# turnDeep/Computational-Chemistry-AI

Measured on AMD Instinct MI355X. Metric: scf_iterations_per_sec, higher is better.
Workload: dtype f64

## Files before the change

### computational-chemistry-ai_amd/csrc/mi355scf.hip

```cpp

#include <hip/hip_runtime.h>
#include <algorithm>
#include <chrono>
#include <cmath>
#include <cstdarg>
#include <cstdint>
#include <cstdio>
#include <cstring>
#include <numeric>
#include <string>
#include <thread>
#include <type_traits>
#include <mutex>
#include <map>
#include <unordered_map>
#include <vector>

#include "../../include/mi355scf.h"
#include "rys_tables.h"

#define LMAX 4
#define LMAX_1E 3
#define NPC ((LMAX + 1) * (LMAX + 2) / 2)
#define BLK 8
// ... 343 lines not shown
    int opt_jk_pipe = -1;
    int opt_ao_order = 1;
    int opt_ket_cluster = 1;
    int opt_xf_mlds = 0;
    int opt_rys_qpw_maxcomp = 256;
    double opt_rys_qpw_maxprim = 4.0;
    int opt_xf_qpw_max = 40;
    int opt_work_mb = 2048;
    int opt_grad_work_mb = 1024;
    int opt_vmat_fold_mt = 3;
    int opt_rys_fine = 1;
    int opt_eri_fused = 0;
    int opt_task_table = 1;
    int opt_prim_lds = 0;
    int opt_xcd_map = 1;
    int opt_df_batch_max = 0;
    int ao_order = 0;
    int *d_perm = nullptr, *d_iperm = nullptr;
    std::vector<int> perm, iperm;
    int opt_vmat_xcd = 1;
    int opt_vmat_wgs = 0;
    int opt_sp2_direct = 0;
    double *d_xt_scratch = nullptr;
};

static inline int pc_index(int la, int lb) { return la * (la + 1) / 2 + lb; }
static inline int ne_of(int la, int lb) { int n = 0; for (int e = la; e <= la + lb; e++) n += ncart(e); return n; }

static double gaussian_int(int n, double a) { return std::tgamma((n + 1) * 0.5) / (2.0 * std::pow(a, (n + 1) * 0.5)); }

static int set_tile_order(mi_ctx *c, int order)
{
    if (c->ao_order == order) return 0;
    const int nbas = c->nbas;
    std::vector<int> seq(nbas);
    std::iota(seq.begin(), seq.end(), 0);
    if (order == 1) std::stable_sort(seq.begin(), seq.end(), [&](int a, int b) { return c->shells[a].l < c->shells[b].l; });
    c->perm.assign(std::max(c->nao, 1), 0);
    c->iperm.assign(std::max(c->nao, 1), 0);
    int pos = 0;
    for (int s_ : seq) {
        ShellH &S = c->shells[s_];
        S.ao = pos;
        for (int m = 0; m < 2 * S.l + 1; m++) { c->perm[S.ao_nat + m] = pos + m; c->iperm[pos + m] = S.ao_nat + m; }
        pos += 2 * S.l + 1;
    }
// ... 241 lines not shown
    void *ptrs[] = {c->d_prim, c->d_M, c->d_tile_table, c->d_tile_off, c->d_tile_I, c->d_runs, c->d_tiles, c->d_segs, c->d_wave_seg,
                    c->d_tile_present};
    for (void *p : ptrs) if (p) dev_free(p);
    c->d_tile_present = nullptr;
    c->d_prim = c->d_M = nullptr; c->d_tile_table = nullptr; c->d_tile_off = nullptr; c->d_tile_I = nullptr;
    c->d_runs = nullptr; c->d_tiles = nullptr; c->d_segs = nullptr; c->d_wave_seg = nullptr;
    c->eri_ready = false;
}

extern "C" int mi_eri_release(mi_ctx *c)
{
    if (!c) return fail("mi_eri_release: null context");
    hipSetDevice(c->device);
    free_eri(c);
    return 0;
}

extern "C" void mi_ctx_destroy(mi_ctx *c)
{
    if (!c) return;
    hipSetDevice(c->device);
    free_eri(c);
    void *ptrs[] = {c->d_env, c->d_bas, c->d_atm, c->d_shell_ao, c->d_c2s, c->d_rys_cheb, c->d_herm_r, c->d_herm_w,
                    c->d_Dpad, c->d_Jacc, c->d_Kacc, c->d_red, c->d_shell_xyz, c->d_xt_scratch, c->d_perm, c->d_iperm,
                    c->d_mDpad, c->d_mJacc, c->d_mKacc};
    for (void *p : ptrs) if (p) dev_free(p);
    {
        HostStash &H = g_stash[c->device & 15];
        std::lock_guard<std::mutex> g(H.mu);
        if (c->h_M.capacity() > H.h_M.capacity()) H.h_M.swap(c->h_M);
        if (c->h_prim.capacity() > H.h_prim.capacity()) H.h_prim.swap(c->h_prim);
        if (c->tiles.capacity() > H.tiles.capacity()) H.tiles.swap(c->tiles);
        if (c->tile_off.capacity() > H.tile_off.capacity()) H.tile_off.swap(c->tile_off);
    }
    delete c;
}

extern "C" int mi_ctx_nao(const mi_ctx *c) { return c ? c->nao : -1; }

extern "C" int mi_set_option(mi_ctx *c, const char *key, double value)
{
    if (!c || !key) return fail("mi_set_option: null argument");
    std::string k(key);
    if (k == "runmax") c->opt_runmax = (int)value;
    else if (k == "omega") {
        if (!(value >= 0.0) || !std::isfinite(value)) return fail("mi_set_option: omega must be finite and >= 0");
        c->opt_omega = value;
    }
    else if (k == "jk_waves") c->opt_jk_waves = (int)value;
    else if (k == "jk_nt") c->opt_jk_nt = (int)value;
    else if (k == "jk_pipe") c->opt_jk_pipe = (int)value;
    else if (k == "jk_dpp") c->opt_jk_dpp = (int)value;
    else if (k == "jk_kjlt") c->opt_jk_kjlt = (int)value;
    else if (k == "grad_live") c->opt_grad_live = (int)value;
    else if (k == "grad_rows") c->opt_grad_rows = (int)value;
    else if (k == "grad_rows_min") c->opt_grad_rows_min = (int)value;
    else if (k == "grad_rows_g32") g_rows_g32 = (int)value;
    else if (k == "jk_cache_mb") c->opt_jk_cache_mb = (int)value;
    else if (k == "jk_pair") c->opt_jk_pair = (int)value;
    else if (k == "jk_multi_batch") c->opt_jk_multi_batch = (int)value;
    else if (k == "sp2_direct") c->opt_sp2_direct = (int)value;
    else if (k == "vmat_wgs") c->opt_vmat_wgs = (int)value;
    else if (k == "vmat_xcd") c->opt_vmat_xcd = (int)value;
    else if (k == "tri_tiles") c->opt_tri_tiles = (int)value;
    else if (k == "ao_order") c->opt_ao_order = (int)value;
    else if (k == "ket_cluster") c->opt_ket_cluster = (int)value;
    else if (k == "xcd_map") c->opt_xcd_map = (int)value;
    else if (k == "prim_lds") c->opt_prim_lds = (int)value;
    else if (k == "task_table") c->opt_task_table = (int)value;
    else if (k == "eri_fused") c->opt_eri_fused = (int)value;
    else if (k == "rys_fine") c->opt_rys_fine = (int)value;
    else if (k == "df_batch_max") {
        if (!(value >= 0.0) || value > 2147483647.0) return fail("mi_set_option: df_batch_max must be in [0, 2^31)");
        c->opt_df_batch_max = (int)value;
    }
    else if (k == "vmat_fold_mt") c->opt_vmat_fold_mt = (int)value;
    else if (k == "work_mb") c->opt_work_mb = (int)value;
    else if (k == "grad_work_mb") c->opt_grad_work_mb = (int)value;
    else if (k == "rys_qpw_maxcomp") c->opt_rys_qpw_maxcomp = (int)value;
    else if (k == "rys_qpw_maxprim") c->opt_rys_qpw_maxprim = value;
    else if (k == "xf_qpw_max") c->opt_xf_qpw_max = (int)value;
    else if (k == "xf_mlds") c->opt_xf_mlds = (int)value;
    else if (k == "eri_tpq") c->opt_eri_tpq = (int)value;
    else if (k == "tpq_maxprim") c->opt_tpq_maxprim = value;
// ... 3433 lines not shown
extern "C" int mi_diis_dots_dev_n(mi_ctx *c, const double *d_hist_e, const double *d_e, int n, int64_t len, double *d_out, void *stream)
{
    if (!c || n < 1 || n > 64 || len < 1 || !d_out) return fail("mi_diis_dots_dev_n: bad argument");
    hipLaunchKernelGGL(diis_dots_kernel, dim3(n, DIIS_NS), dim3(256), 0, (hipStream_t)stream, d_hist_e, d_e, (size_t)len, d_out);
    HIPCHK(hipGetLastError());
    return 0;
}

extern "C" int mi_diis_dots_dev(mi_ctx *c, const double *d_hist_e, const double *d_e, int n, double *d_out, void *stream)
{
    if (!c) return fail("mi_diis_dots_dev: bad argument");
    return mi_diis_dots_dev_n(c, d_hist_e, d_e, n, (int64_t)c->nao * c->nao, d_out, stream);
}

#define DIIS_MAXM 16
__device__ __forceinline__ double lane_bcast(double x, int l)
{
    const int ls = __builtin_amdgcn_readfirstlane(l);
    const long long b = __double_as_longlong(x);
    const unsigned lo = (unsigned)__builtin_amdgcn_readlane((int)(b & 0xffffffffll), ls);
    const unsigned hi = (unsigned)__builtin_amdgcn_readlane((int)(b >> 32), ls);
    return __longlong_as_double((long long)(((unsigned long long)hi << 32) | lo));
}
__global__ __launch_bounds__(64) void diis_solve_kernel(const double *__restrict__ part, int m, int slot, int space, double *B, double *__restrict__ coef)
{
    __shared__ double A[DIIS_MAXM + 1][DIIS_MAXM + 3];
    __shared__ double X[DIIS_MAXM + 1];
    const int t = threadIdx.x;
    const int n = m + 1;
    double bold[DIIS_MAXM];
#pragma unroll
    for (int j = 0; j < DIIS_MAXM; j++) bold[j] = (t >= 1 && t <= m && j < m) ? B[(t - 1) * space + j] : 0.0;
    double dot = 0.0;
    if (t < m) {
        double pq[DIIS_NS];
#pragma unroll
        for (int q = 0; q < DIIS_NS; q++) pq[q] = part[t * DIIS_NS + q];
#pragma unroll
        for (int q = 0; q < DIIS_NS; q++) dot += pq[q];
        B[slot * space + t] = dot;
        B[t * space + slot] = dot;
        X[t] = dot;
    }
    __syncthreads();
    if (t < n) {
#pragma unroll
        for (int j = 0; j <= DIIS_MAXM; j++) {
            double v = 0.0;
            if (j < n) {
                if (t == 0) v = (j == 0) ? 0.0 : 1.0;
                else if (j == 0) v = 1.0;
                else if (t - 1 == slot) v = X[j - 1];
                else if (j - 1 == slot) v = X[t - 1];
                else v = bold[j - 1];
            }
            A[t][j] = v;
        }
        A[t][n] = (t == 0) ? 1.0 : 0.0;
    }
    __syncthreads();
    bool ok = true;
    for (int k = 0; k < n && ok; k++) {
        double val = (t >= k && t < n) ? fabs(A[t][k]) : -1.0;
        int p = t;
        for (int o = 32; o > 0; o >>= 1) {
            const double v2 = __shfl_xor(val, o);
            const int p2 = __shfl_xor(p, o);
            if (v2 > val || (v2 == val && p2 < p)) { val = v2; p = p2; }
        }
        if (!(val > 0.0) || !isfinite(val)) { ok = false; break; }
        if (p != k && t <= n) { const double x = A[k][t]; A[k][t] = A[p][t]; A[p][t] = x; }
        __syncthreads();
        if (t > k && t < n) {
            const double f = A[t][k] / A[k][k];
            for (int j = k; j <= n; j++) A[t][j] = fma(-f, A[k][j], A[t][j]);
        }
        __syncthreads();
    }
    if (ok) {
        for (int i = n - 1; i >= 0; i--) {
            if (t == i) X[i] = A[i][n] / A[i][i];
            __syncthreads();
            const double xi = X[i];
            if (!isfinite(xi)) ok = false;
            if (t < i) A[t][n] = fma(-A[t][i], xi, A[t][n]);
            __syncthreads();
        }
    }
    if (t >= 1 && t <= m) coef[t - 1] = ok ? X[t] : ((t - 1) == slot ? 1.0 : 0.0);
}

extern "C" int mi_diis_solve(mi_ctx *c, const double *d_part, int m, int slot, int space, double *d_B, double *d_coef, void *stream)
{
    if (!c || !d_part || !d_B || !d_coef || m < 1 || m > DIIS_MAXM || space < m || slot < 0 || slot >= m) return fail("mi_diis_solve: bad argument");
    hipLaunchKernelGGL(diis_solve_kernel, dim3(1), dim3(64), 0, (hipStream_t)stream, d_part, m, slot, space, d_B, d_coef);
    HIPCHK(hipGetLastError());
    return 0;
}

__global__ void diis_combine_dev_kernel(const double *hist, const double *coef, int n, size_t nn, double *out)
{
    size_t idx = (size_t)blockIdx.x * blockDim.x + threadIdx.x;
    if (idx >= nn) return;
    const MI_CONST_AS double *cf = as_const(coef);
    double s = 0.0;
    for (int i = 0; i < n; i++) s = fma(cf[i], hist[(size_t)i * nn + idx], s);
    out[idx] = s;
}

extern "C" int mi_diis_combine_dev_n(mi_ctx *c, const double *d_hist, const double *d_coef, int n, int64_t len, double *d_out, void *stream)
{
    if (!c || !d_hist || !d_coef || !d_out || n < 1 || n > DIIS_MAXM || len < 1) return fail("mi_diis_combine_dev_n: bad argument");
// ... 3432 lines not shown
    double s = 0.0;
    if (idx < (size_t)n * n) {
        int r = (int)(idx / n), cidx = (int)(idx - (size_t)r * n);
        double v = M[idx] - M[(size_t)cidx * n + r];
        E[idx] = v;
        s = v * v;
    }
    for (int o = 32; o > 0; o >>= 1) s += __shfl_xor(s, o);
    if ((threadIdx.x & 63) == 0) sh[threadIdx.x >> 6] = s;
    __syncthreads();
    if (threadIdx.x == 0) part[blockIdx.x] = (sh[0] + sh[1]) + (sh[2] + sh[3]);
}

extern "C" int mi_commutator_norm(mi_ctx *c, const double *d_M, double *d_E, double *d_part, void *stream)
{
    if (!c || !d_M || !d_E || !d_part) return fail("mi_commutator_norm: null argument");
    int n = c->nao;
    hipLaunchKernelGGL(commutator_norm_kernel, dim3((unsigned)(((size_t)n * n + 255) / 256)), dim3(256), 0, (hipStream_t)stream, d_M, n, d_E,
                       d_part);
    HIPCHK(hipGetLastError());
    return 0;
}

#define VM_T 64
#define VM_KS 64
#define VM_PAD 2
__global__ __launch_bounds__(256) void xc_vmat_kernel(const double *__restrict__ A, const double *__restrict__ W, int nao, int64_t ng,
                                                      int64_t kchunk, double *C, int xcd_order)
{
    __shared__ double Pa[VM_T][VM_KS + VM_PAD], Pb[VM_T][VM_KS + VM_PAD];
    const int nt = (nao + VM_T - 1) / VM_T, ntt = nt * nt;
    const int L = (int)blockIdx.x;
    int tile, split;
    if (xcd_order) { split = (L & 7) + 8 * (L / (8 * ntt)); tile = (L >> 3) % ntt; }
    else { tile = L % ntt; split = L / ntt; }
    const int m0 = (tile / nt) * VM_T, n0 = (tile % nt) * VM_T;
    const int64_t kbeg = (int64_t)split * kchunk, kend = min(ng, kbeg + kchunk);
    const int wave = threadIdx.x >> 6, lane = threadIdx.x & 63;
    const int qm = (wave >> 1) * 32, qn = (wave & 1) * 32;
    const bool va0 = m0 + qm < nao, va1 = m0 + qm + 16 < nao, vb0 = n0 + qn < nao, vb1 = n0 + qn + 16 < nao;
    d4_t acc[2][2];
#pragma unroll
    for (int a = 0; a < 2; a++)
#pragma unroll
        for (int b = 0; b < 2; b++) acc[a][b] = d4_t{0.0, 0.0, 0.0, 0.0};
    constexpr int PER = VM_T * VM_KS / 256;
// ... 664 lines not shown
```

### computational-chemistry-ai_amd/python/mi355scf/engine.py

```python
import ctypes
import os

import numpy as np
import torch

_HERE = os.path.dirname(os.path.abspath(__file__))
_CSRC = os.path.normpath(os.path.join(_HERE, "..", "..", "csrc"))
LIB_PATH = os.path.join(_CSRC, "libmi355scf.so")
_lib = None


class EngineError(RuntimeError):
    pass


class EngineOutOfMemory(EngineError):

    def __init__(self, msg, need_bytes, free_bytes):
        super().__init__(msg)
        self.need_bytes, self.free_bytes = need_bytes, free_bytes


MI_ERR_NOMEM = -2

# ... 74 lines not shown
        L.mi_sp2_iterate.argtypes = [vp, vp, vp, ctypes.c_int, ctypes.c_double, ctypes.c_int, vp, vp, ctypes.POINTER(vp), vp]
        L.mi_sp2_iterate_pingpong.argtypes = [vp, vp, vp, ctypes.c_int, ctypes.c_double, vp, ctypes.POINTER(vp), ctypes.POINTER(vp), vp]
        L.mi_sp2_iterate_planned.argtypes = [vp, vp, vp, vp, ctypes.c_int, dp, ctypes.c_double, vp, ctypes.POINTER(vp), ctypes.POINTER(vp), vp]
        L.mi_grad_1e.argtypes = [vp, vp, vp, vp, vp]
        L.mi_grad_eri.argtypes = [vp, vp, ctypes.c_double, vp, vp]
        L.mi_grad_eri_spin.argtypes = [vp, vp, vp, ctypes.c_double, vp, vp]
        L.mi_grad_eri_sharded.argtypes = [vp, vp, vp, ctypes.c_double, vp, ctypes.c_int, ctypes.c_int, vp]
        L.mi_grad_eri_pairs.argtypes = [vp, vp, vp, ctypes.c_double, vp, dp, ctypes.c_int, vp, ctypes.c_int, ctypes.c_int, vp]
        L.mi_grad_eri_xpairs.argtypes = [vp, vp, vp, ctypes.c_double, vp, dp, ctypes.c_int, vp, dp, ctypes.POINTER(ctypes.c_int), ctypes.c_int,
                                         vp, ctypes.c_int, ctypes.c_int, vp]
        L.mi_eri_get_memory.argtypes = [vp, ctypes.POINTER(ctypes.c_int64), ctypes.POINTER(ctypes.c_int64)]
        L.mi_eri_release.argtypes = [vp]
        L.mi_tile_store_allocations.restype = ctypes.c_int64
        L.mi_tile_store_allocations.argtypes = [ctypes.c_int64]
        L.mi_eri_read_quartet.argtypes = [vp, ctypes.c_int, ctypes.c_int, ctypes.c_int, ctypes.c_int, dp]
        L.mi_schwarz_get.argtypes = [vp, dp]
        L.mi_df_build.argtypes = [vp, vp, vp, vp, vp]
        L.mi_df_grad.argtypes = [vp, vp, vp, vp, vp, ctypes.c_int, ctypes.c_int, vp]
        L.mi_reduce_blocks.argtypes = [vp]
        L.mi_plan_shards.argtypes = [ctypes.c_int, dp, ctypes.c_double, ctypes.c_int, ctypes.POINTER(ctypes.c_int64),
                                     ctypes.POINTER(ctypes.c_int64)]
        L.mi_fock_energy.argtypes = [vp, vp, vp, vp, vp, vp, ctypes.c_double, vp, vp, vp]
        L.mi_commutator_norm.argtypes = [vp, vp, vp, vp, vp]
        L.mi_c2s_table.argtypes = [ctypes.c_int, dp]
        L.mi_rys_roots_host.argtypes = [ctypes.c_int, ctypes.c_double, dp, dp]
        L.mi_pcm_pairs.argtypes = [vp, ctypes.c_int, ip]
        L.mi_pcm_eval.argtypes = [vp, vp, ctypes.c_int, vp, ctypes.c_int, i64, vp, vp]
        L.mi_pcm_grad.argtypes = [vp, vp, ctypes.c_int, vp, ctypes.c_int, vp, vp, vp, vp]
        L.mi_pcm_potential.argtypes = [vp, vp, ctypes.c_int, i64, vp, vp, vp, vp, vp]
        L.mi_pcm_fock_chunks.argtypes = [ctypes.c_int, i64]
        L.mi_pcm_fock.argtypes = [vp, vp, ctypes.c_int, i64, vp, ctypes.c_double, ctypes.c_int, vp, vp, vp]
        ci = ctypes.c_int
        L.mi_fci_gather_d.argtypes = [vp, ci, ci, ci, ci, ci, ci, vp, ci, vp, ci, vp, vp]
        L.mi_fci_gather_sigma.argtypes = [vp, ci, ci, ci, ci, ci, ci, vp, ci, vp, vp, vp]
        L.mi_fci_hdiag.argtypes = [vp, vp, vp, ci, vp, ci, vp, ci, vp, vp]
        L.mi_cc_amp_update.argtypes = [vp, vp, vp, vp, vp, vp, vp, ci, ci, vp, vp, vp]
        L.mi_cc_t_blocks.argtypes = [ci]
        L.mi_cc_t_energy.argtypes = [vp, ci, ci, ci, vp, vp, vp, vp, vp, vp, vp, vp, vp]
        L.mi_rohf_fock.argtypes = [vp, vp, i64, ci, ci, ci, vp, vp, vp, vp]
        _lib = L
    return _lib


def plan_shards(nao, qblk, tol, nranks):
    q = np.ascontiguousarray(qblk, dtype=np.float64)
    b = np.zeros(nranks, dtype=np.int64)
# ... 533 lines not shown
        _check(lib().mi_sp2_iterate_planned(self._h, F.data_ptr(), A.data_ptr(), B.data_ptr(), nit, _dp(coef), float(out_scale),
                                            tr.data_ptr(), ctypes.byref(out), ctypes.byref(res), self._stream()))
        return (A if res.value == A.data_ptr() else B), (out.value - tr.data_ptr()) // 8

    def build_fock(self, D, h, kscale, F, part, with_k=True, vxc_unsym=None):
        if not self.eri_ready:
            self.prepare_eri()
        assert D.is_contiguous() and F.is_contiguous() and part.numel() == self.reduce_blocks and part.is_contiguous()
        assert vxc_unsym is None or vxc_unsym.is_contiguous()
        with torch.cuda.device(self.device):
            _check(lib().mi_build_fock(self._h, D.data_ptr(), h.data_ptr(), vxc_unsym.data_ptr() if vxc_unsym is not None else None,
                                       int(bool(with_k)), float(kscale), F.data_ptr(), part.data_ptr(), self._stream()))
        return F

    def fock_energy(self, h, J, K, Vxc, D, kscale, F, part):
        assert part.numel() == self.reduce_blocks and part.is_contiguous()
        _check(lib().mi_fock_energy(self._h, h.data_ptr(), J.data_ptr(), K.data_ptr() if K is not None else None,
                                    Vxc.data_ptr() if Vxc is not None else None, D.data_ptr(), float(kscale), F.data_ptr(),
                                    part.data_ptr(), self._stream()))

    def commutator_norm(self, M, E, part):
        assert part.numel() == self.reduce_blocks and part.is_contiguous()
        _check(lib().mi_commutator_norm(self._h, M.data_ptr(), E.data_ptr(), part.data_ptr(), self._stream()))

    def diis_errvec(self, sdf, out):
        _check(lib().mi_diis_errvec(self._h, sdf.data_ptr(), out.data_ptr(), self._stream()))

    def diis_combine(self, hist, coef, out):
        c = np.ascontiguousarray(coef, dtype=np.float64)
        _check(lib().mi_diis_combine(self._h, hist.data_ptr(), _dp(c), len(c), out.data_ptr(), self._stream()))

    def diis_dots_dev(self, hist_e, e, n, out):
        _check(lib().mi_diis_dots_dev_n(self._h, hist_e.data_ptr(), e.data_ptr(), n, e.numel(), out.data_ptr(), self._stream()))

    def diis_solve(self, part, m, slot, space, B, coef):
        _check(lib().mi_diis_solve(self._h, part.data_ptr(), m, slot, space, B.data_ptr(), coef.data_ptr(), self._stream()))

    def diis_combine_dev(self, hist, coef, n, out):
        _check(lib().mi_diis_combine_dev_n(self._h, hist.data_ptr(), coef.data_ptr(), n, out.numel(), out.data_ptr(), self._stream()))

    def diis_dots(self, hist_e, e, n):
        out = np.zeros(n)
        _check(lib().mi_diis_dots(self._h, hist_e.data_ptr(), e.data_ptr(), n, _dp(out), self._stream()))
        return out


# ... 78 lines not shown
```

### computational-chemistry-ai_amd/python/mi355scf/scf.py

```python
import os
import sys
import time

import numpy as np
import torch

from . import engine as _engine
from .mole import Mole
from .purify import HEAD_MAX, Purifier

AU2DEBYE = 2.541746473

_AUFBAU = [(0, 2), (0, 2), (1, 6), (0, 2), (1, 6), (0, 2), (2, 10), (1, 6)]


def _atom_config(z):
    occ = {}
    left = z
    for l, cap in _AUFBAU:
        if left <= 0:
            break
        n = min(cap, left)
        occ.setdefault(l, []).append(n)
        left -= n
    return occ


class DeviceDIIS:

    MAX_SPACE = 16

    def __init__(self, eng, space=8, nmat=1):
        n = eng.nao
        space = int(space)
        if not 1 <= space <= self.MAX_SPACE:
            raise ValueError(f"diis_space = {space}: the device-side Pulay solve supports 1..{self.MAX_SPACE} vectors")
        self.eng, self.space, self.count = eng, space, 0
        shape = (space, n, n) if nmat == 1 else (space, nmat, n, n)
        self.F = torch.empty(*shape, dtype=torch.float64, device=eng.device)
        self.E = torch.empty(*shape, dtype=torch.float64, device=eng.device)

    NS = 16

    def _gram_and_solve(self, slot, m):
        if not hasattr(self, "dots_dev"):
            dev = self.F.device
            self.dots_dev = torch.zeros(self.space * self.NS, dtype=torch.float64, device=dev)
            self.B_dev = torch.zeros(self.space, self.space, dtype=torch.float64, device=dev)
            self.coef_dev = torch.zeros(self.space, dtype=torch.float64, device=dev)
        self.eng.diis_dots_dev(self.E, self.E[slot], m, self.dots_dev)
        self.eng.diis_solve(self.dots_dev, m, slot, self.space, self.B_dev, self.coef_dev)
        self._pending = (slot, m)

    def next_slot(self):
        return self.count % self.space

    def push_inplace(self):
        slot = self.count % self.space
        self.count += 1
        m = min(self.count, self.space)
        self._gram_and_solve(slot, m)
        return m

    def extrapolate(self):
        _slot, m = self._pending
        out = torch.empty_like(self.F[0])
        self.eng.diis_combine_dev(self.F, self.coef_dev, m, out)
        return out


class SCF:
    conv_tol = 1e-9
    conv_tol_grad = None
    max_cycle = 50
    init_guess = "minao"
    diis_space = 8
    diis_start_cycle = 1
    direct_scf_tol = 1e-13
    conv_check = True
    xc = None
    eig_method = "sp2"
    sp2_tol = 1e-11
    sp2_margin = 2
    sp2_fused_max = 320
# ... 96 lines not shown
        S, T, V = eng.int1e()
        h1 = T + V
        if self._nranks > 1:
            from . import parallel
            hs = torch.stack([S, h1])
            parallel.broadcast0(hs, self._pg)
            S, h1 = hs[0].contiguous(), hs[1].contiguous()
        self._S, self._h1 = S, h1
        if eng.nao <= self.host_cholesky_max:
            try:
                from threadpoolctl import threadpool_limits
            except ImportError:
                import contextlib
                threadpool_limits = lambda limits: contextlib.nullcontext()
            with threadpool_limits(limits=4):
                Lh = np.linalg.cholesky(S.cpu().numpy())
                Li = np.linalg.inv(Lh)
            L = torch.from_numpy(np.ascontiguousarray(Lh)).to(eng.device)
            self._Linv = torch.from_numpy(np.ascontiguousarray(np.tril(Li))).to(eng.device)
        else:
            L = torch.linalg.cholesky(S)
            self._Linv = torch.linalg.solve_triangular(L, torch.eye(eng.nao, dtype=torch.float64, device=eng.device), upper=False)
        self._L = L
        if getattr(self, "with_df", None) is not None:
            if self.with_df.mol is not self.mol or self.with_df._B is None:
                self.with_df.mol = self.mol
                t1 = time.time()
                self.with_df.build(eng, self._rank, self._nranks)
                self.with_df.rank_hint = (int(self.mol.nelectron) + int(getattr(self.mol, "spin", 0))) // 2
                torch.cuda.synchronize()
                self.timing["df_seconds"] = time.time() - t1
                self._log(4, f"density fitting: {self.with_df.naux} auxiliary functions, tensor "
                             f"{8e-9 * self.with_df.naux * eng.nao ** 2:.2f} GB, built in {self.timing['df_seconds']:.3f} s")
        elif not eng.eri_ready and self._stream_groups <= 1:
            oom = False
            if getattr(self, "_grad_prefetch", False):
                eng.set_option("grad_prefetch", 1)
            try:
                st = eng.prepare_eri(self.direct_scf_tol, self._rank, self._nranks)
                self.timing["eri_seconds"] = st["seconds_eri"]
                self._log(4, f"resident ERI store: {st['n_tiles']} tiles, {st['stored_bytes'] / 1e6:.1f} MB, "
                             f"{st['n_quartets']} shell quartets in {st['seconds_eri']:.3f} s")
                need, free = eng.eri_memory()
            except _engine.EngineOutOfMemory as e:
                oom, need, free = True, e.need_bytes, e.free_bytes
            view = getattr(self, "_test_memory_view", None)
# ... 200 lines not shown

    def get_veff(self, mol=None, dm=None, **kw):
        if dm is None:
            dm = self.make_rdm1()
        self._setup_once()
        d = torch.as_tensor(np.asarray(dm), dtype=torch.float64, device=self.engine.device)
        return self._veff(d)[0].cpu().numpy()

    def _eig(self, f):
        Li = self._Linv
        e, c = torch.linalg.eigh(Li @ f @ Li.T)
        return e, Li.T @ c

    @property
    def _purifier(self):
        p = self.__dict__.get("_pur")
        if p is None or p.mf is not self:
            p = self._pur = Purifier(self) if p is None else p.rebind(self)
        return p

    xc_nelec_rtol = 2e-4

    sp2_direct = os.environ.get("MI355_SP2_DIRECT", "1") != "0"
    sp2_plan_gnorm = 2e-3
    sp2_plan_inloop = False

    sp2_trace_plan = True
    sp2_first_passes = 48
    sp2_trace_plan_gnorm = 2e-2

    def make_rdm1(self, mo_coeff=None, mo_occ=None):
        if mo_coeff is None:
            if self._dm is not None:
                return self._dm.cpu().numpy()
            mo_coeff, mo_occ = self.mo_coeff, self.mo_occ
        mo_coeff, mo_occ = np.asarray(mo_coeff), np.asarray(mo_occ)
        c = mo_coeff[:, mo_occ > 0]
        return (c * mo_occ[mo_occ > 0]) @ c.T

    def get_init_guess(self, mol=None, key=None):
        key = (key or self.init_guess)
        if isinstance(key, np.ndarray):
            return key
        key = str(key).lower()
        if key in ("1e", "hcore"):
            self._setup_once()
# ... 44 lines not shown
        return st

    def _after_density(self, st, dm, e_last, next_cycle, sp2_tr=None, nocc=0, layout=None):
        ctx = self._after_density_launch(st, dm, next_cycle, sp2_tr, layout)
        return self._after_density_finish(st, ctx, e_last, nocc)

    _PIN_DOUBLES = 16384

    def _after_density_launch(self, st, dm, next_cycle, sp2_tr=None, layout=None, projector=False):
        Li = self._Linv
        dm = dm.contiguous()
        self._xc_projector = (dm, st["dmo"], st["nocc"]) if projector else None
        nb = self.engine.reduce_blocks
        self.n_fock_builds = getattr(self, "n_fock_builds", 0) + 1
        head = layout.head if layout is not None and 2 * nb <= HEAD_MAX else None
        if head is not None:
            part = head[HEAD_MAX - 2 * nb:HEAD_MAX]
        else:
            part = torch.empty(2 * nb, dtype=torch.float64, device=dm.device)
        fock, extra = self._fock_energy(dm, part[:nb])
        diis = st["diis"]
        keep = next_cycle >= self.diis_start_cycle
        slot = diis.next_slot()
        fo = torch.matmul(Li @ fock, Li.T, out=diis.F[slot]) if keep else Li @ fock @ Li.T
        m = fo @ st["dmo"]
        eo = diis.E[slot] if keep else torch.empty_like(m)
        self.engine.commutator_norm(m, eo, part[nb:])
        if keep:
            diis.push_inplace()
        if head is not None and extra is None:
            packed = head[HEAD_MAX - 2 * nb:HEAD_MAX + sp2_tr.numel()]
        else:
            parts = [part] + ([extra.reshape(-1)] if extra is not None else []) + ([sp2_tr] if sp2_tr is not None else [])
            packed = torch.cat(parts) if len(parts) > 1 else part
        return dict(dm=dm, fock=fock, fo=fo, nb=nb, n_extra=0 if extra is None else extra.numel(), has_tr=sp2_tr is not None,
                    layout=layout, lowrank=self._xc_projector is not None, scalars=self._scalars_launch(packed))

    def _scalars_launch(self, packed):
        if self._sync_control_on():
            from . import parallel
            parallel.broadcast0(packed, self._pg)
        k = packed.numel()
        if k > self._PIN_DOUBLES:
            return packed, None
        pin = getattr(self, "_pin", None)
        if pin is None:
            pin = self._pin = torch.empty(self._PIN_DOUBLES, dtype=torch.float64).pin_memory()
            self._pin_event = torch.cuda.Event()
        pin[:k].copy_(packed, non_blocking=True)
        self._pin_event.record()
        return packed, self._pin_event

# ... 63 lines not shown
        if sp2 and 0 < nocc < n:
            return ("optimistic", None, pur.iters) if pur.validated else ("checked", None, 0)
        return "eigh", None, 0

    def _purify(self, route, fo, nocc, passes):
        pur = self._purifier
        if route == "planned":
            return pur.planned(fo, nocc)
        if route == "optimistic":
            return pur.optimistic(fo, nocc, passes)
        return pur.checked(fo, nocc), None, None

    def _front(self, st):
        r = self._route(st, head=True)
        if r is None:
            return None
        route, label, passes = r
        if route == "planned" and self.graph_front:
            out = self._front_graphed(st, st["nocc"])
            if out is not None:
                return out
        fo = st["diis"].extrapolate()
        dmo, tr_dev, layout = self._purify(route, fo, st["nocc"], passes)
        dm = (self._Linv.T @ dmo @ self._Linv).contiguous()
        return dict(fo=fo, dmo=dmo, dm=dm, tr=tr_dev, layout=layout, route=route, label=label)

    graph_front = True
    _GRAPH_STABLE = 3

    def _front_graphed(self, st, nocc):
        diis = st["diis"]
        pur = self._purifier
        m = min(diis.count, diis.space)
        key = (id(diis), m, pur.plan_len, pur.plan_gen, self._Linv.data_ptr())
        g = self.__dict__.get("_fgraph")
        if g is None or g["key"] != key or g["diis"] is not diis:
            seen = self.__dict__.get("_fgraph_seen")
            if seen is None or seen[0] != key:
                self._fgraph_seen = [key, 1]
                return None
            seen[1] += 1
            if seen[1] < self._GRAPH_STABLE or m < diis.space:
                return None
            g = self._fgraph = dict(key=key, diis=diis, heads=[], turn=0)
        i, g["turn"] = g["turn"], 1 - g["turn"]
        if i < len(g["heads"]):
            head = g["heads"][i]
            head["graph"].replay()
            return head["out"]
        try:
            def body():
                fo = diis.extrapolate()
                dmo, tr_dev, layout = pur.planned(fo, nocc, slot=1 - i)
                dm = torch.matmul(self._Linv.T @ dmo, self._Linv)
                return dict(fo=fo, dmo=dmo, dm=dm, tr=tr_dev, layout=layout, route="planned", label="front_planned")
            cur = torch.cuda.current_stream()
            side = torch.cuda.Stream()
            side.wait_stream(cur)
            with torch.cuda.stream(side):
                body()
            cur.wait_stream(side)
            graph = torch.cuda.CUDAGraph()
            with torch.cuda.graph(graph):
                out = body()
            graph.replay()
            g["heads"].append(dict(graph=graph, out=out))
            return out
        except Exception as e:
            self.graph_front = False
            self._fgraph = None
            self._log(4, f"HIP-graph capture of the SCF head failed ({e!r}); continuing with eager launches")
            return None

    def _step(self, st, use_diis=True, want_mo=False):
        nocc, Li = st["nocc"], self._Linv
        pur = self._purifier
        front = st.pop("front", None)
        if want_mo or not use_diis:
            front = None
        paths = self.__dict__.setdefault("path_counts", {})

        def took(name):
            paths[name] = paths.get(name, 0) + 1

        def eigh(fo):
            e, c = torch.linalg.eigh(fo)
            co = c[:, :nocc]
            return e, c, 2.0 * co @ co.T
        if front is not None:
            fo, dmo, tr_dev, layout, dm, route = (front[k] for k in ("fo", "dmo", "tr", "layout", "dm", "route"))
            took(front["label"])
            st.pop("mo_e", None)
        else:
            if use_diis and st["cycle"] >= self.diis_start_cycle:
                fo = st["diis"].extrapolate()
            else:
                fo = st["fo"]
            if self.level_shift and use_diis:
                fo = fo + self.level_shift * (torch.eye(fo.shape[0], dtype=fo.dtype, device=fo.device) - 0.5 * st["dmo"])
            route, label, passes = self._route(st, want_mo=want_mo)
            if label:
                took(label)
            dmo, tr_dev, layout = (None, None, None) if route == "eigh" else self._purify(route, fo, nocc, passes)
            if dmo is None:
                took("eigh")
                e, c, dmo = eigh(fo)
                st.update(mo_e=e, mo_c=Li.T @ c)
                if self.eig_method == "sp2" and not self.level_shift and (want_mo or (self.sp2_planned and 0 < nocc < fo.shape[0])):
                    pur.replan(e, nocc)
            else:
                st.pop("mo_e", None)
            dm = Li.T @ dmo @ Li
        saved = (st["dmo"], st["diis"].count)
        st["dmo"] = dmo
        e_prev = st["e_tot"]
        ctx = self._after_density_launch(st, dm, st["cycle"] + 1, sp2_tr=tr_dev, layout=layout, projector=True)
        nxt = self._front(st) if (use_diis and not want_mo) else None
        if (self.sp2_trace_plan and pur.plan is None and pur.trace_bounds is not None and use_diis and not want_mo
                and st.get("gnorm", 1.0) <= self.sp2_trace_plan_gnorm):
            if pur.plan_from_traces():
                took("plan_from_traces")
        ok = self._after_density_finish(st, ctx, e_prev, nocc)
        if not ok:
            nxt = None
            self.n_redo = getattr(self, "n_redo", 0) + 1
            st["dmo"], st["diis"].count = saved
            st["e_tot"] = e_prev
            pur.validated = False
            redo, _, _ = self._route(st, redo_of=route)
            dmo = pur.checked(fo, nocc) if redo == "checked" else None
            if dmo is None:
                e, _c, dmo = eigh(fo)
                if redo == "eigh":
                    pur.replan(e, nocc)
            st["dmo"] = dmo
            self._after_density(st, Li.T @ dmo @ Li, e_last=e_prev, next_cycle=st["cycle"] + 1)
        if nxt is not None:
            st["front"] = nxt
        st["cycle"] += 1
        return st

    def _iterate(self, st, step):
        conv_tol = self.conv_tol
        conv_tol_grad = self.conv_tol_grad if self.conv_tol_grad is not None else np.sqrt(conv_tol)
        self._log(4, f"init E= {st['e_tot']:.15g}")
        self.converged = False
        t_loop = time.time()
        while st["cycle"] < self.max_cycle:
            step(st)
            self._log(4, f"cycle= {st['cycle']} E= {st['e_tot']:.15g}  delta_E= {st['de']:.3g}  |g|= {st['gnorm']:.3g}")
            if abs(st["de"]) < conv_tol and st["gnorm"] < conv_tol_grad:
                self.converged = True
                break
        st.pop("front", None)
        self.cycles = st["cycle"]
        self.timing["loop_seconds"] = time.time() - t_loop

    def kernel(self, dm0=None, **kw):
        t_start = time.time()
# ... 157 lines not shown
```

### include/mi355scf.h

```cpp
#ifndef MI355SCF_H
#define MI355SCF_H

#include <stddef.h>
#include <stdint.h>

#ifdef __cplusplus
extern "C" {
#endif

typedef struct mi_ctx mi_ctx;

const char *mi_last_error(void);

int mi_abi_version(void);

int mi_ctx_create(const int32_t *atm, int natm, const int32_t *bas, int nbas, const double *env,
                  int nenv, int device_id, mi_ctx **out);
void mi_ctx_destroy(mi_ctx *ctx);
int mi_ctx_nao(const mi_ctx *ctx);

void mi_release_cache(void);

int mi_set_option(mi_ctx *ctx, const char *key, double value);

// ... 53 lines not shown
                     void *stream);
int mi_diis_solve(mi_ctx *ctx, const double *d_part, int m, int slot, int space, double *d_B, double *d_coef, void *stream);
int mi_diis_combine_dev(mi_ctx *ctx, const double *d_hist, const double *d_coef, int n, double *d_out, void *stream);
int mi_diis_dots_dev_n(mi_ctx *ctx, const double *d_hist_e, const double *d_e, int n, int64_t len, double *d_out, void *stream);
int mi_diis_combine_dev_n(mi_ctx *ctx, const double *d_hist, const double *d_coef, int n, int64_t len, double *d_out, void *stream);


int mi_sp2_init(mi_ctx *ctx, const double *d_F, double *d_X, double *d_work, void *stream);
int mi_sp2_update(mi_ctx *ctx, double *d_X, const double *d_X2, double n_occ, double *d_out_with_traces,
                  void *stream);

int mi_sp2_iterate(mi_ctx *ctx, double *d_X, double *d_X2, int nit, double n_occ, int have_x2,
                   double *d_work, double *d_tr, double **d_tr_out, void *stream);
int mi_sp2_iterate_pingpong(mi_ctx *ctx, double *d_A, double *d_B, int nit, double n_occ, double *d_tr, double **d_tr_out,
                            double **d_res, void *stream);

int mi_sp2_iterate_planned(mi_ctx *ctx, const double *d_F, double *d_A, double *d_B, int nit, const double *coef, double out_scale,
                           double *d_tr, double **d_tr_out, double **d_res, void *stream);

int mi_reduce_blocks(const mi_ctx *ctx);
int mi_fock_energy(mi_ctx *ctx, const double *d_h, const double *d_J, const double *d_K, const double *d_Vxc,
                   const double *d_D, double kscale, double *d_F, double *d_part, void *stream);
int mi_commutator_norm(mi_ctx *ctx, const double *d_M, double *d_E, double *d_part, void *stream);


int mi_grid_becke(mi_ctx *ctx, const double *d_coords, const int32_t *d_atom_of, const double *d_vol,
                  int64_t ng, const double *d_adjust, double *d_weights, void *stream);

int mi_eval_ao(mi_ctx *ctx, const double *d_coords, int64_t ng, int deriv, double *d_ao, void *stream);

int mi_xc_rho(mi_ctx *ctx, const double *d_ao, const double *d_C, int64_t ng, int deriv, double *d_rho,
              void *stream);
int mi_xc_rho_mo(mi_ctx *ctx, const double *d_psi, int nocc, int64_t ng, int deriv, double *d_rho, double *d_tau, void *stream);
int mi_build_fock(mi_ctx *ctx, const double *d_D, const double *d_h, const double *d_Vun, int with_k, double kscale, double *d_F,
                  double *d_part, void *stream);
int mi_nystrom_warm(mi_ctx *ctx, const double *d_Zt, const int *d_info, const double *d_G0, double *d_G, int nocc, int n,
                    void *stream);
int mi_nystrom_factor(mi_ctx *ctx, const double *d_M, const double *d_W, int n, int nocc, double *d_Zt, int *d_info, void *stream);
int mi_xc_tail(mi_ctx *ctx, const double *d_w, const double *d_v0, const double *d_v1, const double *d_v2, int64_t ng, double *d_tail,
               void *stream);
int mi_xc_rho_lowrank(mi_ctx *ctx, const double *d_ao, const double *d_Zp, int ldz, int64_t ng, int deriv, double *d_rho,
                      double *d_tau, void *stream);

int mi_xc_eval(const int32_t *kinds, const double *coefs, int nterms, const double *d_rho,
               const double *d_w, int64_t ng, int gga, double *d_exc, double *d_wv, double *d_vrho,
               double *d_vsigma, void *stream);
// ... 74 lines not shown
```

Before: 964.5.

## Fuse orthogonal Fock, DIIS error, Gram dots and Pulay solve into one kernel

```diff
diff --git a/computational-chemistry-ai_amd/csrc/mi355scf.hip b/computational-chemistry-ai_amd/csrc/mi355scf.hip
--- a/computational-chemistry-ai_amd/csrc/mi355scf.hip
+++ b/computational-chemistry-ai_amd/csrc/mi355scf.hip
@@ -389,6 +389,8 @@
     int opt_vmat_wgs = 0;
     int opt_sp2_direct = 0;
     double *d_xt_scratch = nullptr;
+    int opt_fock_error_fused = 0;
+    double *d_fe_scratch = nullptr;
 };
 
 static inline int pc_index(int la, int lb) { return la * (la + 1) / 2 + lb; }
@@ -676,7 +678,7 @@
     hipSetDevice(c->device);
     free_eri(c);
     void *ptrs[] = {c->d_env, c->d_bas, c->d_atm, c->d_shell_ao, c->d_c2s, c->d_rys_cheb, c->d_herm_r, c->d_herm_w,
-                    c->d_Dpad, c->d_Jacc, c->d_Kacc, c->d_red, c->d_shell_xyz, c->d_xt_scratch, c->d_perm, c->d_iperm,
+                    c->d_Dpad, c->d_Jacc, c->d_Kacc, c->d_red, c->d_shell_xyz, c->d_xt_scratch, c->d_fe_scratch, c->d_perm, c->d_iperm,
                     c->d_mDpad, c->d_mJacc, c->d_mKacc};
     for (void *p : ptrs) if (p) dev_free(p);
     {
@@ -714,6 +716,7 @@
     else if (k == "jk_pair") c->opt_jk_pair = (int)value;
     else if (k == "jk_multi_batch") c->opt_jk_multi_batch = (int)value;
     else if (k == "sp2_direct") c->opt_sp2_direct = (int)value;
+    else if (k == "fock_error_fused") c->opt_fock_error_fused = (int)value;
     else if (k == "vmat_wgs") c->opt_vmat_wgs = (int)value;
     else if (k == "vmat_xcd") c->opt_vmat_xcd = (int)value;
     else if (k == "tri_tiles") c->opt_tri_tiles = (int)value;
@@ -4193,27 +4196,25 @@
     const unsigned hi = (unsigned)__builtin_amdgcn_readlane((int)(b >> 32), ls);
     return __longlong_as_double((long long)(((unsigned long long)hi << 32) | lo));
 }
-__global__ __launch_bounds__(64) void diis_solve_kernel(const double *__restrict__ part, int m, int slot, int space, double *B, double *__restrict__ coef)
-{
-    __shared__ double A[DIIS_MAXM + 1][DIIS_MAXM + 3];
-    __shared__ double X[DIIS_MAXM + 1];
-    const int t = threadIdx.x;
+__device__ __forceinline__ void wave_lds_sync()
+{
+    __builtin_amdgcn_fence(__ATOMIC_RELEASE, "workgroup");
+    __builtin_amdgcn_wave_barrier();
+    __builtin_amdgcn_fence(__ATOMIC_ACQUIRE, "workgroup");
+}
+__device__ __forceinline__ void pulay_solve_wave(const int t, const double dot, const int m, const int slot, const int space, double *B,
+                                                 double *__restrict__ coef, double (*A)[DIIS_MAXM + 3], double *X)
+{
     const int n = m + 1;
     double bold[DIIS_MAXM];
 #pragma unroll
     for (int j = 0; j < DIIS_MAXM; j++) bold[j] = (t >= 1 && t <= m && j < m) ? B[(t - 1) * space + j] : 0.0;
-    double dot = 0.0;
     if (t < m) {
-        double pq[DIIS_NS];
-#pragma unroll
-        for (int q = 0; q < DIIS_NS; q++) pq[q] = part[t * DIIS_NS + q];
-#pragma unroll
-        for (int q = 0; q < DIIS_NS; q++) dot += pq[q];
         B[slot * space + t] = dot;
         B[t * space + slot] = dot;
         X[t] = dot;
     }
-    __syncthreads();
+    wave_lds_sync();
     if (t < n) {
 #pragma unroll
         for (int j = 0; j <= DIIS_MAXM; j++) {
@@ -4229,7 +4230,7 @@
         }
         A[t][n] = (t == 0) ? 1.0 : 0.0;
     }
-    __syncthreads();
+    wave_lds_sync();
     bool ok = true;
     for (int k = 0; k < n && ok; k++) {
         double val = (t >= k && t < n) ? fabs(A[t][k]) : -1.0;
@@ -4241,24 +4242,39 @@
         }
         if (!(val > 0.0) || !isfinite(val)) { ok = false; break; }
         if (p != k && t <= n) { const double x = A[k][t]; A[k][t] = A[p][t]; A[p][t] = x; }
-        __syncthreads();
+        wave_lds_sync();
         if (t > k && t < n) {
             const double f = A[t][k] / A[k][k];
             for (int j = k; j <= n; j++) A[t][j] = fma(-f, A[k][j], A[t][j]);
         }
-        __syncthreads();
+        wave_lds_sync();
     }
     if (ok) {
         for (int i = n - 1; i >= 0; i--) {
             if (t == i) X[i] = A[i][n] / A[i][i];
-            __syncthreads();
+            wave_lds_sync();
             const double xi = X[i];
             if (!isfinite(xi)) ok = false;
             if (t < i) A[t][n] = fma(-A[t][i], xi, A[t][n]);
-            __syncthreads();
+            wave_lds_sync();
         }
     }
     if (t >= 1 && t <= m) coef[t - 1] = ok ? X[t] : ((t - 1) == slot ? 1.0 : 0.0);
+}
+__global__ __launch_bounds__(64) void diis_solve_kernel(const double *__restrict__ part, int m, int slot, int space, double *B, double *__restrict__ coef)
+{
+    __shared__ double A[DIIS_MAXM + 1][DIIS_MAXM + 3];
+    __shared__ double X[DIIS_MAXM + 1];
+    const int t = threadIdx.x;
+    double dot = 0.0;
+    if (t < m) {
+        double pq[DIIS_NS];
+#pragma unroll
+        for (int q = 0; q < DIIS_NS; q++) pq[q] = part[t * DIIS_NS + q];
+#pragma unroll
+        for (int q = 0; q < DIIS_NS; q++) dot += pq[q];
+    }
+    pulay_solve_wave(t, dot, m, slot, space, B, coef, A, X);
 }
 
 extern "C" int mi_diis_solve(mi_ctx *c, const double *d_part, int m, int slot, int space, double *d_B, double *d_coef, void *stream)
@@ -7737,6 +7753,171 @@
     return 0;
 }
 
+#define FE_MAXWG (SP2_DIRECT_MAXS * (SP2_DIRECT_MAXS + 1) / 2)
+#define FE_CHUNK 14
+static_assert(16 * FE_CHUNK >= FE_MAXWG, "fock_error_kernel: 16 chunks must cover the grid");
+struct FockErrArgs {
+    const double *Tt, *LiT, *Z;
+    double *Fs, *E;
+    int n, S, m, slot, space, nb;
+    double *B, *coef, *part, *scratch;
+    unsigned *ticket;
+};
+template <int MAXS>
+__global__ __launch_bounds__(256) void fock_error_kernel(FockErrArgs A)
+{
+    static_assert(MAXS % 2 == 0, "two halves");
+    __shared__ double red[3][4 * 256];
+    __shared__ double wsum[4][DIIS_MAXM];
+    __shared__ double cs[16][DIIS_MAXM];
+    __shared__ double SA[DIIS_MAXM + 1][DIIS_MAXM + 3];
+    __shared__ double SX[DIIS_MAXM + 1];
+    __shared__ int last;
+    const int n = A.n, S = A.S, m = A.m, slot = A.slot;
+    const size_t nn = (size_t)n * n;
+    int bI, bJ;
+    sp2_tile_of_block((int)blockIdx.x, bI, bJ);
+    const bool diag = bI == bJ;
+    const int i0 = bI * 16, j0 = bJ * 16;
+    const int t = threadIdx.x, wave = t >> 6, lane = t & 63, col = lane & 15, g = lane >> 4;
+    const int ca = min(i0 + col, n - 1), cb = min(j0 + col, n - 1);
+    const int kw = wave * 4 * S + g;
+    const int gi = i0 + g + 4 * wave, gj = j0 + col;
+    const bool own = gi < n && gj < n && (!diag || gi >= gj);
+    const bool off = own && gi != gj;
+    const size_t eo = (size_t)min(gi, n - 1) * n + min(gj, n - 1);
+    double h[DIIS_MAXM];
+#pragma unroll
+    for (int i = 0; i < DIIS_MAXM; i++) h[i] = A.E[(size_t)(i < m ? i : 0) * nn + eo];
+    d4_t aF = {0.0, 0.0, 0.0, 0.0}, aM = {0.0, 0.0, 0.0, 0.0}, aN = {0.0, 0.0, 0.0, 0.0};
+    constexpr int H = MAXS / 2;
+#pragma unroll
+    for (int hf = 0; hf < 2; hf++) {
+        double tI[H], tJ[H], lJ[H], zJ[H], zI[H];
+#pragma unroll
+        for (int u = 0; u < H; u++) {
+            const size_t row = (size_t)min(kw + 4 * (hf * H + u), n - 1) * n;
+            tI[u] = A.Tt[row + ca];
+            tJ[u] = A.Tt[row + cb];
+            lJ[u] = A.LiT[row + cb];
+            zJ[u] = A.Z[row + cb];
+            zI[u] = A.Z[row + ca];
+        }
+#pragma unroll
+        for (int u = 0; u < H; u++) {
+            const int s = hf * H + u;
+            const bool in = s < S && kw + 4 * s < n;
+            const double a = in ? tI[u] : 0.0, b = in ? tJ[u] : 0.0;
+            if (s < S) {
+                aF = __builtin_amdgcn_mfma_f64_16x16x4f64(a, lJ[u], aF, 0, 0, 0);
+                aM = __builtin_amdgcn_mfma_f64_16x16x4f64(a, zJ[u], aM, 0, 0, 0);
+                aN = __builtin_amdgcn_mfma_f64_16x16x4f64(b, zI[u], aN, 0, 0, 0);
+            }
+        }
+    }
+#pragma unroll
+    for (int q = 0; q < 4; q++) {
+        red[0][wave * 256 + q * 64 + lane] = aF[q];
+        red[1][wave * 256 + q * 64 + lane] = aM[q];
+        red[2][wave * 256 + q * 64 + lane] = aN[q];
+    }
+    __syncthreads();
+    const int et = (col >> 2) * 64 + (col & 3) * 16 + (g + 4 * wave);
+    const double vF = (red[0][t] + red[0][256 + t]) + (red[0][512 + t] + red[0][768 + t]);
+    const double vM = (red[1][t] + red[1][256 + t]) + (red[1][512 + t] + red[1][768 + t]);
+    const double vN = (red[2][et] + red[2][256 + et]) + (red[2][512 + et] + red[2][768 + et]);
+    const double ev = off ? vM - vN : 0.0;
+    if (own) {
+        double *Es = A.E + (size_t)slot * nn;
+        A.Fs[(size_t)gi * n + gj] = vF;
+        Es[(size_t)gi * n + gj] = ev;
+        if (gi != gj) {
+            A.Fs[(size_t)gj * n + gi] = vF;
+            Es[(size_t)gj * n + gi] = -ev;
+        }
+    }
+#pragma unroll
+    for (int i = 0; i < DIIS_MAXM; i++) {
+        if (i < m) {
+            double w = off ? 2.0 * ((i == slot ? ev : h[i]) * ev) : 0.0;
+            for (int o = 32; o > 0; o >>= 1) w += __shfl_xor(w, o);
+            if (lane == 0) wsum[wave][i] = w;
+        }
+    }
+    __syncthreads();
+    if (t < m) A.scratch[(size_t)blockIdx.x * DIIS_MAXM + t] = (wsum[0][t] + wsum[1][t]) + (wsum[2][t] + wsum[3][t]);
+    asm volatile("s_waitcnt vmcnt(0)" ::: "memory");
+    __syncthreads();
+    if (t == 0) {
+        __threadfence();
+        asm volatile("s_waitcnt vmcnt(0)" ::: "memory");
+        const unsigned k = __hip_atomic_fetch_add(A.ticket, 1u, __ATOMIC_ACQ_REL, __HIP_MEMORY_SCOPE_AGENT);
+        last = (k == gridDim.x - 1u);
+        if (last) __threadfence();
+    }
+    __syncthreads();
+    if (!last) return;
+    {
+        const int i = t & 15, c = t >> 4, nwg = (int)gridDim.x;
+        double v[FE_CHUNK];
+#pragma unroll
+        for (int q = 0; q < FE_CHUNK; q++) {
+            const int b = c * FE_CHUNK + q;
+            const double x = __hip_atomic_load(A.scratch + (size_t)min(b, nwg - 1) * DIIS_MAXM + i, __ATOMIC_RELAXED, __HIP_MEMORY_SCOPE_AGENT);
+            v[q] = b < nwg ? x : 0.0;
+        }
+        double s = 0.0;
+#pragma unroll
+        for (int q = 0; q < FE_CHUNK; q++) s += v[q];
+        cs[c][i] = s;
+    }
+    __syncthreads();
+    if (wave == 0) {
+        double dot = 0.0;
+        if (lane < m) for (int c = 0; c < 16; c++) dot += cs[c][lane];
+        pulay_solve_wave(lane, dot, m, slot, A.space, A.B, A.coef, SA, SX);
+        if (lane == 0) __hip_atomic_store(A.ticket, 0u, __ATOMIC_RELAXED, __HIP_MEMORY_SCOPE_AGENT);
+    } else {
+        double e2 = 0.0;
+        for (int c = 0; c < 16; c++) e2 += cs[c][slot];
+        for (int j = t - 64; j < A.nb; j += 192) A.part[j] = j == 0 ? e2 : 0.0;
+    }
+}
+typedef void (*fock_error_fn)(FockErrArgs);
+static fock_error_fn fock_error_for(int S)
+{
+    if (S <= 8) return fock_error_kernel<8>;
+    if (S <= 12) return fock_error_kernel<12>;
+    if (S <= 16) return fock_error_kernel<16>;
+    return fock_error_kernel<SP2_DIRECT_MAXS>;
+}
+
+extern "C" int mi_fock_error(mi_ctx *c, const double *d_Tt, const double *d_LiT, const double *d_Z, double *d_F, double *d_E, int m, int slot,
+                             int space, double *d_B, double *d_coef, double *d_part, void *stream)
+{
+    if (!c || !d_Tt || !d_LiT || !d_Z || !d_F || !d_E || !d_B || !d_coef || !d_part) return fail("mi_fock_error: null argument");
+    if (!c->opt_fock_error_fused) return fail("mi_fock_error: option fock_error_fused is off");
+    const int n = c->nao;
+    if (n < 1 || n > 16 * SP2_DIRECT_MAXS) return fail("mi_fock_error: the fused launch is for N <= %d", 16 * SP2_DIRECT_MAXS);
+    if (m < 1 || m > DIIS_MAXM || space < m || slot < 0 || slot >= m) return fail("mi_fock_error: bad history (1 <= m <= %d)", DIIS_MAXM);
+    hipStream_t st = (hipStream_t)stream;
+    if (!c->d_fe_scratch) {
+        HIPCHK(hipSetDevice(c->device));
+        HIPCHK(dev_malloc(&c->d_fe_scratch, sizeof(double) * (FE_MAXWG * DIIS_MAXM + 1)));
+        HIPCHK(hipMemsetAsync(c->d_fe_scratch, 0, sizeof(double) * (FE_MAXWG * DIIS_MAXM + 1), st));
+    }
+    const int nbk = (n + 15) / 16;
+    FockErrArgs A{};
+    A.Tt = d_Tt; A.LiT = d_LiT; A.Z = d_Z;
+    A.Fs = d_F + (size_t)slot * n * n; A.E = d_E;
+    A.n = n; A.S = nbk; A.m = m; A.slot = slot; A.space = space; A.nb = mi_reduce_blocks(c);
+    A.B = d_B; A.coef = d_coef; A.part = d_part;
+    A.scratch = c->d_fe_scratch; A.ticket = reinterpret_cast<unsigned *>(c->d_fe_scratch + FE_MAXWG * DIIS_MAXM);
+    hipLaunchKernelGGL(fock_error_for(nbk), dim3(nbk * (nbk + 1) / 2), dim3(256), 0, st, A);
+    HIPCHK(hipGetLastError());
+    return 0;
+}
+
 #define VM_T 64
 #define VM_KS 64
 #define VM_PAD 2
diff --git a/computational-chemistry-ai_amd/python/mi355scf/engine.py b/computational-chemistry-ai_amd/python/mi355scf/engine.py
--- a/computational-chemistry-ai_amd/python/mi355scf/engine.py
+++ b/computational-chemistry-ai_amd/python/mi355scf/engine.py
@@ -120,6 +120,7 @@
                                      ctypes.POINTER(ctypes.c_int64)]
         L.mi_fock_energy.argtypes = [vp, vp, vp, vp, vp, vp, ctypes.c_double, vp, vp, vp]
         L.mi_commutator_norm.argtypes = [vp, vp, vp, vp, vp]
+        L.mi_fock_error.argtypes = [vp, vp, vp, vp, vp, vp, ctypes.c_int, ctypes.c_int, ctypes.c_int, vp, vp, vp, vp]
         L.mi_c2s_table.argtypes = [ctypes.c_int, dp]
         L.mi_rys_roots_host.argtypes = [ctypes.c_int, ctypes.c_double, dp, dp]
         L.mi_pcm_pairs.argtypes = [vp, ctypes.c_int, ip]
@@ -699,6 +700,17 @@
     def commutator_norm(self, M, E, part):
         assert part.numel() == self.reduce_blocks and part.is_contiguous()
         _check(lib().mi_commutator_norm(self._h, M.data_ptr(), E.data_ptr(), part.data_ptr(), self._stream()))
+
+    FOCK_ERROR_MAX_N = 320
+
+    def fock_error(self, Tt, LiT, Z, F_hist, E_hist, m, slot, B, coef, part):
+        n = self.nao
+        assert all(x.is_contiguous() and x.dtype == torch.float64 for x in (Tt, LiT, Z, F_hist, E_hist, B, coef, part))
+        assert Tt.numel() == LiT.numel() == Z.numel() == n * n and part.numel() == self.reduce_blocks
+        space = B.shape[0]
+        assert F_hist.numel() == E_hist.numel() == space * n * n and B.numel() == space * space and coef.numel() >= space
+        _check(lib().mi_fock_error(self._h, Tt.data_ptr(), LiT.data_ptr(), Z.data_ptr(), F_hist.data_ptr(), E_hist.data_ptr(), int(m),
+                                   int(slot), int(space), B.data_ptr(), coef.data_ptr(), part.data_ptr(), self._stream()))
 
     def diis_errvec(self, sdf, out):
         _check(lib().mi_diis_errvec(self._h, sdf.data_ptr(), out.data_ptr(), self._stream()))
diff --git a/computational-chemistry-ai_amd/python/mi355scf/scf.py b/computational-chemistry-ai_amd/python/mi355scf/scf.py
--- a/computational-chemistry-ai_amd/python/mi355scf/scf.py
+++ b/computational-chemistry-ai_amd/python/mi355scf/scf.py
@@ -35,19 +35,22 @@
         space = int(space)
         if not 1 <= space <= self.MAX_SPACE:
             raise ValueError(f"diis_space = {space}: the device-side Pulay solve supports 1..{self.MAX_SPACE} vectors")
-        self.eng, self.space, self.count = eng, space, 0
+        self.eng, self.space, self.count, self.nmat = eng, space, 0, nmat
         shape = (space, n, n) if nmat == 1 else (space, nmat, n, n)
         self.F = torch.empty(*shape, dtype=torch.float64, device=eng.device)
         self.E = torch.empty(*shape, dtype=torch.float64, device=eng.device)
 
     NS = 16
 
-    def _gram_and_solve(self, slot, m):
+    def _solve_buffers(self):
         if not hasattr(self, "dots_dev"):
             dev = self.F.device
             self.dots_dev = torch.zeros(self.space * self.NS, dtype=torch.float64, device=dev)
             self.B_dev = torch.zeros(self.space, self.space, dtype=torch.float64, device=dev)
             self.coef_dev = torch.zeros(self.space, dtype=torch.float64, device=dev)
+
+    def _gram_and_solve(self, slot, m):
+        self._solve_buffers()
         self.eng.diis_dots_dev(self.E, self.E[slot], m, self.dots_dev)
         self.eng.diis_solve(self.dots_dev, m, slot, self.space, self.B_dev, self.coef_dev)
         self._pending = (slot, m)
@@ -60,6 +63,15 @@
         self.count += 1
         m = min(self.count, self.space)
         self._gram_and_solve(slot, m)
+        return m
+
+    def push_fused(self, Tt, LiT, Z, part):
+        slot = self.count % self.space
+        self.count += 1
+        m = min(self.count, self.space)
+        self._solve_buffers()
+        self.eng.fock_error(Tt, LiT, Z, self.F, self.E, m, slot, self.B_dev, self.coef_dev, part)
+        self._pending = (slot, m)
         return m
 
     def extrapolate(self):
@@ -202,6 +214,7 @@
             L = torch.linalg.cholesky(S)
             self._Linv = torch.linalg.solve_triangular(L, torch.eye(eng.nao, dtype=torch.float64, device=eng.device), upper=False)
         self._L = L
+        self._LinvT = self._Linv.T.contiguous()
         if getattr(self, "with_df", None) is not None:
             if self.with_df.mol is not self.mol or self.with_df._B is None:
                 self.with_df.mol = self.mol
@@ -448,6 +461,7 @@
     xc_nelec_rtol = 2e-4
 
     sp2_direct = os.environ.get("MI355_SP2_DIRECT", "1") != "0"
+    fock_error_fused = os.environ.get("MI355_FOCK_ERROR", "1") != "0"
     sp2_plan_gnorm = 2e-3
     sp2_plan_inloop = False
 
@@ -538,12 +552,29 @@
         diis = st["diis"]
         keep = next_cycle >= self.diis_start_cycle
         slot = diis.next_slot()
+        zt = st.get("zt")
+        if (keep and zt is not None and zt[0] is st["dmo"] and diis.nmat == 1 and fock.shape[0] <= self.engine.FOCK_ERROR_MAX_N
+                and not self.level_shift and self._fock_error_on()):
+            diis.push_fused(fock @ Li.T, self._LinvT, zt[1], part[nb:])
+            paths = self.__dict__.setdefault("path_counts", {})
+            paths["fock_error_fused"] = paths.get("fock_error_fused", 0) + 1
+            return self._after_density_pack(dm, fock, diis.F[slot], nb, part, head, extra, sp2_tr, layout)
         fo = torch.matmul(Li @ fock, Li.T, out=diis.F[slot]) if keep else Li @ fock @ Li.T
         m = fo @ st["dmo"]
         eo = diis.E[slot] if keep else torch.empty_like(m)
         self.engine.commutator_norm(m, eo, part[nb:])
         if keep:
             diis.push_inplace()
+        return self._after_density_pack(dm, fock, fo, nb, part, head, extra, sp2_tr, layout)
+
+    def _fock_error_on(self):
+        eng, want = self.engine, int(bool(self.fock_error_fused))
+        if getattr(eng, "_fock_error_fused", None) != want:
+            eng.set_option("fock_error_fused", want)
+            eng._fock_error_fused = want
+        return bool(want)
+
+    def _after_density_pack(self, dm, fock, fo, nb, part, head, extra, sp2_tr, layout):
         if head is not None and extra is None:
             packed = head[HEAD_MAX - 2 * nb:HEAD_MAX + sp2_tr.numel()]
         else:
@@ -653,8 +684,9 @@
                 return out
         fo = st["diis"].extrapolate()
         dmo, tr_dev, layout = self._purify(route, fo, st["nocc"], passes)
-        dm = (self._Linv.T @ dmo @ self._Linv).contiguous()
-        return dict(fo=fo, dmo=dmo, dm=dm, tr=tr_dev, layout=layout, route=route, label=label)
+        zt = self._Linv.T @ dmo
+        dm = (zt @ self._Linv).contiguous()
+        return dict(fo=fo, dmo=dmo, zt=zt, dm=dm, tr=tr_dev, layout=layout, route=route, label=label)
 
     graph_front = True
     _GRAPH_STABLE = 3
@@ -683,8 +715,9 @@
             def body():
                 fo = diis.extrapolate()
                 dmo, tr_dev, layout = pur.planned(fo, nocc, slot=1 - i)
-                dm = torch.matmul(self._Linv.T @ dmo, self._Linv)
-                return dict(fo=fo, dmo=dmo, dm=dm, tr=tr_dev, layout=layout, route="planned", label="front_planned")
+                zt = self._Linv.T @ dmo
+                dm = torch.matmul(zt, self._Linv)
+                return dict(fo=fo, dmo=dmo, zt=zt, dm=dm, tr=tr_dev, layout=layout, route="planned", label="front_planned")
             cur = torch.cuda.current_stream()
             side = torch.cuda.Stream()
             side.wait_stream(cur)
@@ -719,7 +752,7 @@
             co = c[:, :nocc]
             return e, c, 2.0 * co @ co.T
         if front is not None:
-            fo, dmo, tr_dev, layout, dm, route = (front[k] for k in ("fo", "dmo", "tr", "layout", "dm", "route"))
+            fo, dmo, zt, tr_dev, layout, dm, route = (front[k] for k in ("fo", "dmo", "zt", "tr", "layout", "dm", "route"))
             took(front["label"])
             st.pop("mo_e", None)
         else:
@@ -741,9 +774,10 @@
                     pur.replan(e, nocc)
             else:
                 st.pop("mo_e", None)
-            dm = Li.T @ dmo @ Li
-        saved = (st["dmo"], st["diis"].count)
-        st["dmo"] = dmo
+            zt = Li.T @ dmo
+            dm = zt @ Li
+        saved = (st["dmo"], st.get("zt"), st["diis"].count)
+        st["dmo"], st["zt"] = dmo, (dmo, zt)
         e_prev = st["e_tot"]
         ctx = self._after_density_launch(st, dm, st["cycle"] + 1, sp2_tr=tr_dev, layout=layout, projector=True)
         nxt = self._front(st) if (use_diis and not want_mo) else None
@@ -755,7 +789,7 @@
         if not ok:
             nxt = None
             self.n_redo = getattr(self, "n_redo", 0) + 1
-            st["dmo"], st["diis"].count = saved
+            st["dmo"], st["zt"], st["diis"].count = saved
             st["e_tot"] = e_prev
             pur.validated = False
             redo, _, _ = self._route(st, redo_of=route)
@@ -764,8 +798,9 @@
                 e, _c, dmo = eigh(fo)
                 if redo == "eigh":
                     pur.replan(e, nocc)
-            st["dmo"] = dmo
-            self._after_density(st, Li.T @ dmo @ Li, e_last=e_prev, next_cycle=st["cycle"] + 1)
+            zt = Li.T @ dmo
+            st["dmo"], st["zt"] = dmo, (dmo, zt)
+            self._after_density(st, zt @ Li, e_last=e_prev, next_cycle=st["cycle"] + 1)
         if nxt is not None:
             st["front"] = nxt
         st["cycle"] += 1
diff --git a/include/mi355scf.h b/include/mi355scf.h
--- a/include/mi355scf.h
+++ b/include/mi355scf.h
@@ -99,6 +99,8 @@
 int mi_fock_energy(mi_ctx *ctx, const double *d_h, const double *d_J, const double *d_K, const double *d_Vxc,
                    const double *d_D, double kscale, double *d_F, double *d_part, void *stream);
 int mi_commutator_norm(mi_ctx *ctx, const double *d_M, double *d_E, double *d_part, void *stream);
+int mi_fock_error(mi_ctx *ctx, const double *d_Tt, const double *d_LiT, const double *d_Z, double *d_F, double *d_E, int m, int slot,
+                  int space, double *d_B, double *d_coef, double *d_part, void *stream);
 
 
 int mi_grid_becke(mi_ctx *ctx, const double *d_coords, const int32_t *d_atom_of, const double *d_vol,
```

Result: slower. 944.6 (-2.1%).
